# terra-render/Terra

Measured on AMD Instinct MI355X. Metric: Msamples/s, higher is better.
Workload: dtype f32; 1 GPU; cornell_1080p_512spp; scene=cornell32, width=1920, height=1080, spp=512, bounces=8, integrator=simple, triangles=32, tree=auto, traversal=reference tree + leaf-box cull, tile=64, sample_split=8, parallelism=single

## Files before the change

### terra_amd/csrc/integrators_device.h

```cpp
#pragma once
#include "shading_device.h"

TD float randf ( Pcg32& b, Counters& c, int count ) { if ( count == 2 ) ++c.rand_calls; return trng_b_float ( b ); }

TD float triangle_area ( V3 a, V3 b, V3 cc ) { return length ( cross ( b - a, cc - a ) ) / 2; }

struct LightSample { uint32_t light_object; uint32_t tri_in_object; uint32_t tri; float pick_pdf; V3 pos, norm; };

template <int COUNT, int MODE = 0>
TD LightSample draw_light_sample ( const DevScene& sc, Pcg32& rb, Counters& c, const Tracer* T = nullptr ) {
    LightSample ls;
    float e = ( float ) ( ( double ) randf ( rb, c, COUNT ) - 1e-4 );
    double xl = ( double ) e * ( double ) sc.n_lights;
    uint32_t li = xl < 0 ? 0u : ( uint32_t ) xl;
    ls.pick_pdf = 1.f / ( float ) sc.lights_triangles_count;
    DevLight l = ( MODE == 1 && T ) ? T->l_lights[li] : sc.lights[li];
    float e_t = randf ( rb, c, COUNT );
    uint32_t k = ( uint32_t ) ( e_t * ( float ) l.tri_count );
    if ( k >= l.tri_count ) k = l.tri_count - 1;
    ls.light_object = l.object; ls.tri_in_object = k; ls.tri = l.first_tri + k;
    float e1 = randf ( rb, c, COUNT ), e2 = randf ( rb, c, COUNT );
    const float4* tris = ( MODE == 1 && T ) ? reinterpret_cast<const float4*> ( T->l_tris ) : reinterpret_cast<const float4*> ( sc.tris );
    const float4* props = ( MODE == 1 && T ) ? T->l_props : reinterpret_cast<const float4*> ( sc.props );
    V3 ta, tb, tc; tri_vertices ( tris, ls.tri, ta, tb, tc );
// ... 279 lines not shown
    } else if ( INTEGRATOR == 2 ) {
        return integrate_mis<COUNT, MODE, KINDS, false> ( T, sf, p, wo, throughput, bounce, rb, c );
    } else if ( INTEGRATOR == 3 ) {
        return bounce != 0 ? v3 ( 0, 0, 0 ) : v3 ( 1, 1, 1 );
    } else if ( INTEGRATOR == 4 ) {
        if ( bounce != 0 ) return v3 ( 0, 0, 0 );
        float d = length ( ray.o - p ) / 500.f;
        return v3 ( d, d, d );
    } else if ( INTEGRATOR == 5 ) {
        return integrate_debug_normals ( sf, bounce );
    } else {
        return integrate_mis<COUNT, MODE, KINDS, true> ( T, sf, p, wo, throughput, bounce, rb, c );
    }
}

template <int COUNT>
TD PathDraws path_draw ( const float2* sincos24, Pcg32& rb, Counters& c ) {
    PathDraws d;
    d.e0 = randf ( rb, c, COUNT ); d.e1 = randf ( rb, c, COUNT ); d.e2 = randf ( rb, c, COUNT );
    d.az = azimuth_fetch ( sincos24, d.e1 );
    d.e3 = randf ( rb, c, COUNT );
    return d;
}
template <int KINDS>
TD bool path_continue ( Surface& sf, V3 wo, V3& throughput, uint32_t& bounce, uint32_t max_bounces, const PathDraws& d, V3& wi ) {
    wi = bsdf_sample<KINDS> ( sf, d.e0, d.e1, d.e2, wo, d.az );
    float pdf = sel_max ( bsdf_pdf<KINDS> ( sf, wi, wo ), ( float ) 1e-4 );
    V3 f = bsdf_eval<KINDS> ( sf, wi, wo ) * rcp_exact ( pdf );
    throughput = had ( throughput, f );
    throughput = throughput * dot ( sf.normal, wi );
    float pr = sel_max ( throughput.x, sel_max ( throughput.y, throughput.z ) );
    if ( d.e3 > pr ) return false;
        throughput = throughput * roulette_scale ( pr );
    ++bounce;
    return bounce <= max_bounces;
}
// ... 78 lines not shown
```

### terra_amd/csrc/render_kernels.hip

```cpp
#include <hip/hip_runtime.h>
#include "trace_device.h"
#include "kernels.h"
#include "launch_plan.h"
#include "empty_proof.h"

#ifdef TERRA_TU
#define TERRA_TU_HAS(k) ( TERRA_TU == ( k ) )
#define TERRA_TU_MODE(k) ( TERRA_TU == ( k ) || TERRA_TU == ( k ) + 4 || TERRA_TU == ( k ) + 8 || TERRA_TU == ( k ) + 12 )
#else
#define TERRA_TU_HAS(k) ( !TERRA_RAY_SOURCE )
#define TERRA_TU_MODE(k) 1
#endif
#if TERRA_RAY_SOURCE == 3
typedef DevPointRenderParams RenderKernelParams;
#elif TERRA_RAY_SOURCE == 2
typedef DevLensRenderParams RenderKernelParams;
#elif TERRA_RAY_SOURCE == 1
typedef DevRayRenderParams RenderKernelParams;
#else
typedef DevRenderParams RenderKernelParams;
#endif

struct DevResult { float acc[3]; int samples; };

// ... 612 lines not shown
    while ( true ) {
        const bool any_alive = __any ( alive );
        if ( !alive && ( TERRA_REGEN_MIN <= 1 || !any_alive || __popcll ( __ballot ( !alive ) ) >= TERRA_REGEN_MIN ) ) {
            if ( jb.s == p.chunk_spp && ( TERRA_JOB_FETCH_MIN <= 1 || !any_alive || __popcll ( __ballot ( jb.s == p.chunk_spp ) ) >= TERRA_JOB_FETCH_MIN ) ) TERRA_JOB_NEXT();
            if ( jb.exhausted ) break;
            if ( jb.s != p.chunk_spp ) {
                PS_WAVE ( c, kPsCamIter ); PS_LANE ( c, kPsCamLanes );
                float r1 = trng_a_float ( rs.a ), r2 = trng_a_float ( rs.a );
                TERRA_PRIMARY_RAY ( ro, rd, r1, r2 );
                if constexpr ( ( KINDS & TERRA_KIND_SAMPLER ) != 0 ) sp = sampler_pair_draw ( p.sampler_mode, p.sampler_strata, ( uint64_t ) jb.base + jb.s, rs.a );
                TERRA_LENS_RAY ( ro, rd, r1, r2 );
                lo_reset(); throughput = v3 ( 1, 1, 1 ); bounce = 0; alive = true; ++jb.s;
            }
        }
        if ( alive ) {
            ray = make_ray ( ro, rd );
            Surface sf;
            PS_WAVE ( c, kPsRayIter ); PS_LANE ( c, kPsRayLanes );
            constexpr bool pre_draw = !TERRA_IS_LIGHT ( INTEGRATOR );
            PathDraws pd;
            RaycastResult h = scene_raycast<COUNT, MODE, KINDS> ( T, ray, sf, c, pre_draw ? &pd : nullptr, pre_draw ? &rs.b : nullptr );
            bool end = !h.hit;
            if ( h.hit ) {
                PS_WAVE ( c, kPsShadeIter ); PS_LANE ( c, kPsShadeLanes );
                V3 wo = neg ( ray.d ), wi;
                constexpr bool SPLIT_DIRECT = INTEGRATOR == 1 && ( KINDS & ( TERRA_KIND_TEX | TERRA_KIND_SAMPLER ) ) == 0;
                if constexpr ( SPLIT_DIRECT ) {
                    Ray shadow_ray;
                    const DirectPending pend = direct_prepare<COUNT, KINDS, MODE> ( T, sf, h.point, wo, throughput, bounce, rs.b, c, shadow_ray );
                    pd = path_draw<COUNT> ( T.sc.sincos24, rs.b, c );
                    end = !path_continue<KINDS> ( sf, wo, throughput, bounce, p.bounces, pd, wi );
                    if ( !end ) { ro = surface_origin ( sf, h.point ); rd = wi; }
                    const uint32_t tri = scene_raycast_triangle<COUNT, MODE> ( T, shadow_ray, c, pend.expected );
                    lo_add ( tri == pend.expected ? pend.vis : pend.hid );
                } else if constexpr ( INTEGRATOR == 2 && ( KINDS & ( TERRA_KIND_TEX | TERRA_KIND_SAMPLER ) ) == 0 ) {
                    Ray ray_a; V3 b_d;
                    const MisPending pend = mis_prepare<COUNT, KINDS, MODE> ( T, sf, h.point, wo, throughput, bounce, rs.b, c, ray_a, b_d );
                    const V3 next_o = surface_origin ( sf, h.point );
                    end = !path_continue<COUNT, KINDS> ( T.sc, sf, wo, throughput, bounce, p.bounces, rs.b, c, wi, sp );
                    if ( !end ) { ro = next_o; rd = wi; }
                    const uint32_t tri_a = scene_raycast_triangle<COUNT, MODE> ( T, ray_a, c, pend.expected );
                    const V3 lo_a = tri_a == pend.expected ? pend.a_vis : pend.a_hid;
                    Surface lsf;
                    const RaycastResult hb = scene_raycast<COUNT, MODE, KINDS> ( T, make_ray ( next_o, b_d ), lsf, c );
                    lo_add ( mis_finish_b<MODE> ( T, pend, lo_a, hb.hit, hb.object, hb.tri, hb.point, lsf, b_d ) );
                } else {
                lo_add ( integrate<INTEGRATOR, COUNT, MODE, KINDS> ( T, ray, sf, h.point, wo, throughput, bounce, rs.b, c ) );
                if ( !pre_draw ) pd = path_draw<COUNT> ( T.sc.sincos24, rs.b, c );
                if constexpr ( ( KINDS & TERRA_KIND_SAMPLER ) != 0 ) path_apply_sampler ( pd, sp, bounce );
                end = !path_continue<KINDS> ( sf, wo, throughput, bounce, p.bounces, pd, wi );
                if ( !end ) { ro = surface_origin ( sf, h.point ); rd = wi; }
                }
            } else if ( ( KINDS & TERRA_KIND_ENV ) && T.sc.env_mode && !env_reaches_by_samples<INTEGRATOR, KINDS> ( T.sc, bounce ) ) {
                throughput = had ( throughput, environment_eval ( T.sc, ray.d ) );
                lo_add ( throughput );
            }
            if ( end ) { lo_deposit(); alive = false; }
        }
    }
    }

    if ( COUNT ) wave_flush_counters ( c, p.counters );
    if ( COUNT == 2 && p.leaf_cull ) {
// ... 309 lines not shown
```

### terra_amd/csrc/rng.h

```cpp
#pragma once
#include <stdint.h>

#if defined(__HIPCC__)
#define TRNG_FN __host__ __device__ inline
#else
#define TRNG_FN static inline
#endif

struct Pcg32 { uint64_t state, inc; };

TRNG_FN uint64_t trng_splitmix64 ( uint64_t z ) {
    z += 0x9E3779B97F4A7C15ull;
    z = ( z ^ ( z >> 30 ) ) * 0xBF58476D1CE4E5B9ull;
    z = ( z ^ ( z >> 27 ) ) * 0x94D049BB133111EBull;
    return z ^ ( z >> 31 );
}

TRNG_FN uint32_t trng_next ( Pcg32& g ) {
    uint64_t old = g.state;
    g.state = old * 6364136223846793005ull + g.inc;
    uint32_t xs = ( uint32_t ) ( ( ( old >> 18 ) ^ old ) >> 27 );
    uint32_t rot = ( uint32_t ) ( old >> 59 );
    return ( xs >> rot ) | ( xs << ( ( 0u - rot ) & 31u ) );
}
// ... 10 lines not shown

TRNG_FN PixelStreams trng_pixel_streams ( uint64_t frame_seed, uint64_t pix, uint64_t samples_so_far ) {
    PixelStreams s;
    uint64_t k = trng_splitmix64 ( trng_splitmix64 ( frame_seed + pix ) ^ ( samples_so_far * 0x9E3779B97F4A7C15ull ) );
    s.seedA = ( uint32_t ) ( k >> 32 );
    s.a.state = 0; s.a.inc = 1;
    trng_next ( s.a );
    s.a.state += s.seedA;
    trng_next ( s.a );
    trng_seed ( s.b, trng_splitmix64 ( k ^ 1ull ), trng_splitmix64 ( k ^ 2ull ) );
    return s;
}

TRNG_FN float trng_a_float ( Pcg32& a ) { return ( float ) trng_next ( a ) * 0x1p-32f; }
TRNG_FN float trng_b_float ( Pcg32& b ) { return ( float ) ( trng_next ( b ) >> 8 ) * 0x1p-24f; }
```

### terra_amd/csrc/shading_device.h

```cpp
#pragma once
#include "traverse_fast.h"

TD float texture_coord ( float u ) { return u > -1.f ? fminf ( u, 4294967040.f ) : 0.f; }
TD V3 texture_read ( const DevTexture& t, uint32_t x, uint32_t y ) {
    const uint32_t W = t.width, H = t.height;
    if ( t.address_mode == 2 ) { x = x < W - 1 ? x : W - 1; y = y < H - 1 ? y : H - 1; }
    else if ( t.address_mode == 0 ) { x %= W; y %= H; }
    else if ( ( x / W ) % 2 == 0 ) { x %= W; y %= H; }
    else { x = W - ( x % W ); y = H - ( y % H ); x = x < W - 1 ? x : W - 1; y = y < H - 1 ? y : H - 1; }
    const size_t e = ( ( size_t ) y * W + x ) * t.components;
    if ( t.depth == 1 ) {
        const uint8_t* p = reinterpret_cast<const uint8_t*> ( t.data ) + e;
        return v3 ( p[0] / 255.f, p[1] / 255.f, p[2] / 255.f );
    }
    const float* p = reinterpret_cast<const float*> ( t.data ) + e;
    return v3 ( p[0], p[1], p[2] );
}
TD V3 texture_sample ( const DevTexture& t, float u, float v ) {
    u = texture_coord ( u ); v = texture_coord ( v );
    uint32_t ix = ( uint32_t ) u, iy = ( uint32_t ) v;
    if ( t.filter == 0 ) return texture_read ( t, ix, iy );
    if ( t.filter != 1 ) return v3 ( 0, 0, 0 );
    uint32_t x2 = ix + 1 < t.width - 1 ? ix + 1 : t.width - 1, y2 = iy + 1 < t.height - 1 ? iy + 1 : t.height - 1;
    V3 n1 = texture_read ( t, ix, iy ), n2 = texture_read ( t, x2, iy ), n3 = texture_read ( t, ix, y2 ), n4 = texture_read ( t, x2, y2 );
// ... 73 lines not shown
        float tx = ( pc2.x * v + pb2.x * u ) + pa2.x * w;
        float ty = ( pc2.y * v + pb2.y * u ) + pa2.y * w;
        #pragma unroll
        for ( int i = 0; i < 4; ++i ) if ( m.tex[i] >= 0 ) sf.attr[i] = texture_sample ( T.sc.textures[m.tex[i]], tx, ty );
        if ( m.tex[TERRA_DEV_MAX_ATTR] >= 0 ) sf.emissive = texture_sample ( T.sc.textures[m.tex[TERRA_DEV_MAX_ATTR]], tx, ty );
    }
    sf.bsdf = m.bsdf;
    sf.ior = m.ior;
    nattr_out = m.attributes_count;
}

struct RaycastResult { bool hit; uint32_t object, tri_in_object, tri; V3 point; };

struct Azimuth { float sn, cs; bool have; };
struct PathDraws { float e0, e1, e2, e3; Azimuth az; };
template <int COUNT> TD PathDraws path_draw ( const float2* sincos24, Pcg32& rb, Counters& c );

template <int COUNT, int MODE, int KINDS>
TD RaycastResult scene_raycast ( const Tracer& T, const Ray& in, Surface& sf, Counters& c, PathDraws* pre = nullptr, Pcg32* rb = nullptr ) {
    Ray r = in;
    r.o = r.o + r.d * 0.001f;
    RayState st = ray_state_init ( r );
    if ( COUNT ) ++c.rays;
    Closest best;
    if ( MODE >= 2 ) { ClosestRanked b2 = bvh_traverse_fast<COUNT, MODE == 3> ( T, r, st, c ); best.depth = b2.depth; best.tri = b2.tri; }
    else best = bvh_traverse<COUNT, MODE> ( T, r, st, c );
    RaycastResult res; res.hit = best.tri != 0xffffffffu; res.tri = best.tri; res.object = 0; res.tri_in_object = 0;
    res.point = res.hit ? r.o + r.d * best.depth : v3 ( FLT_MAX, FLT_MAX, FLT_MAX );
    if ( res.hit ) {
        uint32_t nattr;
        if ( pre ) *pre = path_draw<COUNT> ( T.sc.sincos24, *rb, c );
        surface_init<MODE, KINDS> ( T, best.tri, res.point, sf, res.object, res.tri_in_object, nattr );
        if ( MODE >= 2 ) res.tri = T.sc.mats[res.object].first_tri + res.tri_in_object;
        if ( COUNT ) ++c.hits;
        if ( COUNT == 2 ) c.attr_fetches += nattr + 1;
    }
    return res;
}

template <int COUNT, int MODE>
TD uint32_t scene_raycast_triangle ( const Tracer& T, const Ray& in, Counters& c, uint32_t expected ) {
    Ray r = in;
    r.o = r.o + r.d * 0.001f;
    RayState st = ray_state_init ( r );
    if ( COUNT ) ++c.rays;
    if constexpr ( MODE == 2 && COUNT == 0 ) {
        const V3 o_perm = permuted ( r.o, st );
        ClosestRanked best;
        if ( !fast_expect ( T, st, o_perm, expected, best ) ) return 0xffffffffu;
        int* top = T.stack; uint32_t hand = TERRA_FAST_ROOT_IN_HAND, held = 0u;
        traverse_fast_resume<COUNT> ( T, r, st, o_perm, best, top, hand, held, 0, c, false, true );
        return best.tri == TERRA_TRI_EXPECTED ? expected : 0xffffffffu;
    }
    if constexpr ( MODE == 1 && COUNT == 0 ) {
        const V3 o_perm = permuted ( r.o, st );
        float depth;
        if ( !watertight_permuted ( tri_perm_lds ( T.l_tris + 12 * expected, st ), o_perm, st, depth ) ) return 0xffffffffu;
        Closest best; best.depth = __uint_as_float ( __float_as_uint ( depth + 0.f ) + 1u ); best.tri = 0xffffffffu;
        if ( T.pairs ) { best.depth = depth; best.tri = terra_pair_key ( __float_as_uint ( T.l_tris[12 * expected + 11] ), expected ); }
        if ( T.fused && __all ( ray_is_tame ( r ) ) ) traverse_loops<COUNT, MODE, true, true, true> ( T, r, st, o_perm, best, c, expected );
        else if ( __all ( ray_is_regular ( r ) ) ) traverse_loops<COUNT, MODE, true, false, true> ( T, r, st, o_perm, best, c, expected );
        else traverse_loops<COUNT, MODE, false, false, true> ( T, r, st, o_perm, best, c, expected );
        if ( T.pairs ) return best.tri != 0u ? expected : 0xffffffffu;
        return best.tri;
    }
    uint32_t tri;
    if ( MODE >= 2 ) { const ClosestRanked b2 = bvh_traverse_fast<COUNT, MODE == 3> ( T, r, st, c ); tri = b2.tri; }
    else tri = bvh_traverse<COUNT, MODE> ( T, r, st, c ).tri;
    if ( tri == 0xffffffffu ) return tri;
    uint32_t object;
// ... 9 lines not shown
    return tri;
}

TD V3 surface_origin ( const Surface& sf, V3 p ) { return p + sf.normal * 0.0001f; }
TD Ray surface_ray ( const Surface& sf, V3 p, V3 d ) { return make_ray ( surface_origin ( sf, p ), d ); }


TD Azimuth azimuth_none() { Azimuth a; a.sn = 0.f; a.cs = 1.f; a.have = false; return a; }
TD Azimuth azimuth_fetch ( const float2* tab, float e ) {
    Azimuth a = azimuth_none();
    const float x = e * 16777216.f;
    if ( tab && e >= 0.f && x < 16777216.f ) {
        const uint32_t k = ( uint32_t ) x;
        if ( ( float ) k == x ) { const float2 v = tab[k]; a.cs = v.x; a.sn = v.y; a.have = true; }
    }
    return a;
}
TD void azimuth_sincos ( const Azimuth& az, float e, float& sn, float& cs ) {
    if ( az.have ) { sn = az.sn; cs = az.cs; }
    else tdm_sincosf_pair ( 2 * TERRA_PI_F * e, sn, cs );
}

TD V3 diffuse_sample ( const Surface& sf, float e1, float e2, const Azimuth& az ) {
    float r = sqrt_exact ( e1 );
    float sn, cs;
    azimuth_sincos ( az, e2, sn, cs );
    float x = r * cs;
    float z = r * sn;
    V3 wi = v3 ( x, sqrt_exact ( sel_max ( 0.f, 1 - e1 ) ), z );
    return normalize ( basis_apply ( make_basis ( sf.normal ), wi ) );
// ... 145 lines not shown
```

### terra_amd/csrc/trace_geometry.h

```cpp
#pragma once
#include "trace_math.h"

TD void camera_film ( const DevRenderParams& p, uint32_t px, uint32_t py, float r1, float r2, float& sx, float& sy ) {
    float dx = -p.jitter + 2 * r1 * p.jitter;
    float dy = -p.jitter + 2 * r2 * p.jitter;
    float ndc_x, ndc_y; div2_exact_rk ( ( float ) px + 0.5f + dx, ( float ) py + 0.5f + dy, ( float ) p.fb_w, p.inv_fb_w, ( float ) p.fb_h, p.inv_fb_h, ndc_x, ndc_y );
    sx = 2 * ndc_x - 1;
    sy = 1 - 2 * ndc_y;
}
TD V3 camera_rotate ( const DevRenderParams& p, V3 d ) {
    return v3 ( p.cam_rot[0] * d.x + p.cam_rot[1] * d.y + p.cam_rot[2] * d.z,
                p.cam_rot[3] * d.x + p.cam_rot[4] * d.y + p.cam_rot[5] * d.z,
                p.cam_rot[6] * d.x + p.cam_rot[7] * d.y + p.cam_rot[8] * d.z );
}
TD V3 camera_sample ( const DevRenderParams& p, uint32_t px, uint32_t py, float r1, float r2 ) {
    float sx, sy; camera_film ( p, px, py, r1, r2, sx, sy );
    float fx = sx * p.aspect * p.tan_half_fov;
    float fy = sy * p.tan_half_fov;
    V3 d = normalize ( v3 ( fx, fy, 1.f ) );
    return camera_rotate ( p, d );
}

TD void concentric_disk ( float l1, float l2, float& u, float& v ) {
    const float kPi2 = tdm_float ( 0x3FC90FDBu ), kPi4 = tdm_float ( 0x3F490FDBu );
// ... 129 lines not shown
}

TD RayState ray_state_init ( const Ray& r ) {
    float ax = fabsf ( r.d.x ), ay = fabsf ( r.d.y ), az = fabsf ( r.d.z );
    int iz = ax > ay ? ( ax > az ? 0 : 2 ) : ( ay > az ? 1 : 2 );
    int ix = iz + 1 == 3 ? 0 : iz + 1;
    int iy = ix + 1 == 3 ? 0 : ix + 1;
    if ( pick ( r.d, iz ) < 0.f ) { int t = ix; ix = iy; iy = t; }
    RayState s;
    s.scalez = pick ( r.inv, iz );
    s.shearx = pick ( r.d, ix ) * s.scalez;
    s.sheary = pick ( r.d, iy ) * s.scalez;
    s.ix = ix; s.iy = iy; s.iz = iz;
    return s;
}

TD void tri_vertices ( float4 t0, float4 t1, float4 t2, V3& a, V3& b, V3& c ) { a = v3 ( t0.x, t0.y, t0.z ); b = v3 ( t1.x, t1.y, t1.z ); c = v3 ( t2.x, t2.y, t2.z ); }
TD void tri_vertices ( const float4* tris, uint32_t i, V3& a, V3& b, V3& c ) { tri_vertices ( tris[3 * i], tris[3 * i + 1], tris[3 * i + 2], a, b, c ); }

struct TriPerm { float a[3], b[3], c[3]; };
TD TriPerm tri_perm_lds ( const float* t, const RayState& s ) {
    TriPerm p;
    p.a[0] = t[s.ix]; p.a[1] = t[s.iy]; p.a[2] = t[s.iz];
    p.b[0] = t[4 + s.ix]; p.b[1] = t[4 + s.iy]; p.b[2] = t[4 + s.iz];
    p.c[0] = t[8 + s.ix]; p.c[1] = t[8 + s.iy]; p.c[2] = t[8 + s.iz];
    return p;
}
TD TriPerm tri_perm ( float4 t0, float4 t1, float4 t2, const RayState& s ) {
    const V3 va = v3 ( t0.x, t0.y, t0.z ), vb = v3 ( t1.x, t1.y, t1.z ), vc = v3 ( t2.x, t2.y, t2.z );
    TriPerm p;
// ... 138 lines not shown
```

### terra_amd/csrc/trace_math.h

```cpp
#pragma once
#include <hip/hip_runtime.h>
#include <float.h>
#include "dev_types.h"
#include "dev_math.h"
#include "rng.h"
#include "sampling_device.h"
#include "exact_div.h"
#include "exact_sqrt.h"

#define TD __device__ __forceinline__

struct V3 { float x, y, z; };

TD V3 v3 ( float x, float y, float z ) { V3 r; r.x = x; r.y = y; r.z = z; return r; }
TD V3 v3p ( const float* p ) { return v3 ( p[0], p[1], p[2] ); }
TD V3 operator+ ( V3 a, V3 b ) { return v3 ( a.x + b.x, a.y + b.y, a.z + b.z ); }
TD V3 operator- ( V3 a, V3 b ) { return v3 ( a.x - b.x, a.y - b.y, a.z - b.z ); }
TD V3 operator* ( V3 a, float s ) { return v3 ( a.x * s, a.y * s, a.z * s ); }
TD V3 had ( V3 a, V3 b ) { return v3 ( a.x * b.x, a.y * b.y, a.z * b.z ); }
TD V3 neg ( V3 a ) { return v3 ( -a.x, -a.y, -a.z ); }
TD float dot ( V3 a, V3 b ) { return a.x * b.x + a.y * b.y + a.z * b.z; }
TD V3 cross ( V3 a, V3 b ) { return v3 ( a.y * b.z - a.z * b.y, a.z * b.x - a.x * b.z, a.x * b.y - a.y * b.x ); }
TD float length2 ( V3 a ) { return a.x * a.x + a.y * a.y + a.z * a.z; }
TD float length ( V3 a ) { return sqrtf ( length2 ( a ) ); }
// ... 25 lines not shown
    } else {
        float k = sqrtf ( n.y * n.y + n.z * n.z );
        t = v3 ( 0.f * k, -n.z * k, n.y * k );
    }
    return basis_of ( t, n );
}
TD Basis make_basis ( V3 n ) {
    const bool c = fabsf ( n.x ) > fabsf ( n.y );
    const float a = c ? n.x : n.y;
    const float k = sqrt_exact ( a * a + n.z * n.z );
    return basis_of ( v3 ( ( c ? n.z : 0.f ) * k, ( c ? 0.f : -n.z ) * k, ( c ? -n.x : n.y ) * k ), n );
}

struct Ray { V3 o, d, inv; };
TD Ray make_ray ( V3 o, V3 d ) { Ray r; r.o = o; r.d = d; rcp3_exact ( d.x, d.y, d.z, r.inv.x, r.inv.y, r.inv.z ); return r; }

struct RayState { float shearx, sheary, scalez; int ix, iy, iz; };
TD V3 permuted ( V3 a, const RayState& s ) { return v3 ( pick ( a, s.ix ), pick ( a, s.iy ), pick ( a, s.iz ) ); }
```

### terra_amd/csrc/traverse_ref.h

```cpp
#pragma once
#include "trace_geometry.h"
#include <stddef.h>

#ifndef TERRA_PHASE_STATS
#define TERRA_PHASE_STATS 0
#endif
struct Counters {
    uint32_t rays, nodes, tri_tests, hits, rand_calls, attr_fetches;
    uint32_t tri_culled;
#if TERRA_PHASE_STATS
    uint32_t ps[16];
#endif
};
TD Counters counters_zero() {
    Counters c; c.rays = c.nodes = c.tri_tests = c.hits = c.rand_calls = c.attr_fetches = c.tri_culled = 0;
#if TERRA_PHASE_STATS
    for ( int i = 0; i < 16; ++i ) c.ps[i] = 0;
#endif
    return c;
}
#if TERRA_PHASE_STATS
#define PS_WAVE(c, k) do { if ( ( int ) ( threadIdx.x & 63 ) == __ffsll ( ( long long ) __ballot ( 1 ) ) - 1 ) ++( c ).ps[k]; } while ( 0 )
#define PS_LANE(c, k) do { ++( c ).ps[k]; } while ( 0 )
#else
// ... 164 lines not shown
    uint32_t sx = r.inv.x < 0.f ? kNeg : 0u, sy = r.inv.y < 0.f ? kNeg : 0u, sz = r.inv.z < 0.f ? kNeg : 0u;
    asm ( "" : "+v" ( sx ), "+v" ( sy ), "+v" ( sz ) );
    uint32_t bx = table + kX + sx, by = table + kY + sy, bz = table + kZ + sz;
    asm ( "" : "+v" ( bx ), "+v" ( by ), "+v" ( bz ) );
    const char* pm = reinterpret_cast<const char*> ( T.l_props ) + terra_leaf_box_mask_offset ( 0 );
    uint32_t leaf_set = 0u, entry = 0u;
    if constexpr ( PAIRS ) nb.lo = nb.hi = TERRA_NO_BOX;
    #pragma clang loop vectorize(disable) interleave(disable) unroll(disable)
    for ( uint32_t g = T.n_boxes / TERRA_LEAF_BOX_GROUP; g != 0; --g ) leaf_box_group<TERRA_LEAF_BOX_GROUP, kStride, PAIRS> ( bx, by, bz, pm, r, sel, leaf_set, c, entry, nb );
    if ( T.n_boxes & 4u ) leaf_box_group<4, kStride, PAIRS> ( bx, by, bz, pm, r, sel, leaf_set, c, entry, nb );
    #pragma clang loop vectorize(disable) interleave(disable) unroll(disable)
    for ( uint32_t k = T.n_boxes % 4u; k != 0; --k ) leaf_box_group<1, kStride, PAIRS> ( bx, by, bz, pm, r, sel, leaf_set, c, entry, nb );
    return leaf_set;
}

template <int COUNT, int MODE, bool FAST, bool FUSED, bool ANYHIT>
TD void traverse_pairs ( const Tracer& T, const Ray& r, const RayState& st, V3 o_perm, Closest& best, Counters& c ) {
    const SlabSel sel = slab_sel ( r );
    uint32_t leaf_set = 0u;
    PS_WAVE ( c, kPsDrainIter );
    bool flat = false;
    if constexpr ( FUSED ) flat = T.n_boxes != 0u;
    NearestBoxes nb; nb.lo = nb.hi = TERRA_NO_BOX;
    bool nearest = false;
    if ( flat ) { leaf_set = leaf_boxes_flat<true> ( T, r, sel, c, nb ); nearest = T.nearest; }
    else {
        int* sp = T.stack; int* lp = nullptr;
        *sp = 0; sp += TERRA_COL;
        while ( sp != T.stack ) node_step<COUNT, MODE, FAST, FUSED, true> ( T, r, sel, sp, lp, leaf_set, c );
    }
    const uint32_t perm = 2u * ( uint32_t ) st.iz + ( uint32_t ) ( st.ix != ( st.iz == 2 ? 0 : st.iz + 1 ) );
    const float4* copy = T.l_ranked + ( TERRA_PAIR_ENTRY_BYTES / 16 ) * ( T.lds_tris >> 1 ) * perm;
    float depth_best = best.depth; uint32_t key_best = ANYHIT ? best.tri : 0u;
    bool beaten = false;
    const float cut = __uint_as_float ( ( uint32_t ) ( nearest ? nb.hi : TERRA_NO_BOX ) & ~31u );
    if ( ANYHIT && nearest && depth_best < __uint_as_float ( ( uint32_t ) nb.lo & ~31u ) ) leaf_set = 0u;
    uint32_t next = nearest ? ( uint32_t ) nb.lo & 31u : ( uint32_t ) __builtin_ctz ( leaf_set | 0x80000000u );
    while ( leaf_set != 0u ) {
        PS_WAVE ( c, kPsLeafIter ); PS_LANE ( c, kPsLeafLanes );
        const float4* e = copy + ( TERRA_PAIR_ENTRY_BYTES / 16 ) * next;
        leaf_set &= ~ ( 1u << next );
        const uint2 keys = *reinterpret_cast<const uint2*> ( e + 3 );
        auto load = [&] ( bool again ) {
            uint32_t a = ( uint32_t ) ( uintptr_t ) e;
            if ( again ) asm volatile ( "" : "+v" ( a ) );
            typedef float Piece __attribute__ (( ext_vector_type ( 4 ) ));
// ... 3 lines not shown
        };
        watertight_pair ( load, o_perm, st, [&] ( float depth, bool second ) {
            const uint32_t key = second ? keys.y : keys.x;
            if ( ( depth < depth_best ) | ( ( depth == depth_best ) & ( key < key_best ) ) ) {
                if ( ANYHIT ) { beaten = true; leaf_set = 0u; }
                else { depth_best = depth; key_best = key; }
            }
        } );
        if ( depth_best < cut ) leaf_set = 0u;
        next = ( uint32_t ) __builtin_ctz ( leaf_set | 0x80000000u );
    }
    best.depth = depth_best;
    best.tri = ANYHIT ? ( beaten ? 0u : key_best ) : ( key_best ? ( key_best & 31u ) : 0xffffffffu );
}

template <int COUNT, int MODE, bool FAST, bool FUSED = false, bool ANYHIT = false>
TD void traverse_ranked ( const Tracer& T, const Ray& r, const RayState& st, V3 o_perm, Closest& best, Counters& c, uint32_t expected ) {
    if constexpr ( COUNT == 0 ) if ( T.pairs ) { traverse_pairs<COUNT, MODE, FAST, FUSED, ANYHIT> ( T, r, st, o_perm, best, c ); return; }
    const SlabSel sel = slab_sel ( r );
    uint32_t leaf_set = 0u;
    PS_WAVE ( c, kPsDrainIter );
    bool flat = false;
    if constexpr ( COUNT == 0 && FUSED ) flat = T.n_boxes != 0u;
    NearestBoxes no_nb;
    if ( flat ) leaf_set = leaf_boxes_flat<false> ( T, r, sel, c, no_nb );
    else {
        int* sp = T.stack; int* lp = nullptr;
        *sp = 0; sp += TERRA_COL;
        while ( sp != T.stack ) node_step<COUNT, MODE, FAST, FUSED, true> ( T, r, sel, sp, lp, leaf_set, c );
    }
    const uint32_t perm = 2u * ( uint32_t ) st.iz + ( uint32_t ) ( st.ix != ( st.iz == 2 ? 0 : st.iz + 1 ) );
    const float4* copy = T.l_ranked + 3u * T.lds_tris * perm;
    while ( leaf_set != 0u ) {
        PS_WAVE ( c, kPsLeafIter ); PS_LANE ( c, kPsLeafLanes );
        const float4* e = copy + 3u * ( uint32_t ) __builtin_ctz ( leaf_set );
        leaf_set &= leaf_set - 1u;
        const float4 q0 = e[0], q1 = e[1], q2 = e[2];
        const TriPerm tp = { { q0.x, q0.y, q0.z }, { q0.w, q1.x, q1.y }, { q1.z, q1.w, q2.x } };
        if ( COUNT ) ++c.tri_tests;
        float depth;
        if ( watertight_permuted ( tp, o_perm, st, depth ) && depth < best.depth ) {
            const uint32_t ti = __float_as_uint ( q2.y );
            best.depth = depth; best.tri = ti;
            if ( ANYHIT && ti != expected ) leaf_set = 0u;
        }
    }
}

template <int COUNT, int MODE, bool FAST, bool FUSED = false, bool ANYHIT = false>
TD void traverse_loops ( const Tracer& T, const Ray& r, const RayState& st, V3 o_perm, Closest& best, Counters& c, uint32_t expected = 0xffffffffu ) {
    if constexpr ( MODE == 1 ) if ( T.ranked ) { traverse_ranked<COUNT, MODE, FAST, FUSED, ANYHIT> ( T, r, st, o_perm, best, c, expected ); return; }
    const SlabSel sel = slab_sel ( r );
    int* sp = T.stack; int* lp = T.leaves;
    int* const lp_full = T.leaves + ( T.leaf_cap - 2 ) * TERRA_COL;
    uint32_t no_set = 0u;
    *sp = 0; sp += TERRA_COL;
    for ( ;; ) {
        PS_WAVE ( c, kPsDrainIter );
        while ( sp != T.stack && lp <= lp_full ) node_step<COUNT, MODE, FAST, FUSED> ( T, r, sel, sp, lp, no_set, c );
        if constexpr ( ANYHIT ) {
            bool stop = false;
            for ( const int* e = T.leaves; e != lp && !stop; e += TERRA_COL ) leaf_step<COUNT, MODE, true> ( T, e, st, o_perm, best, c, expected, &stop );
            if ( stop ) sp = T.stack;
        } else
        for ( const int* e = T.leaves; e != lp; e += TERRA_COL ) leaf_step<COUNT, MODE> ( T, e, st, o_perm, best, c );
        lp = T.leaves;
        if ( sp == T.stack ) break;
    }
}

template <int COUNT, int MODE>
TD Closest bvh_traverse ( const Tracer& T, const Ray& r, const RayState& st, Counters& c ) {
    Closest best; best.depth = FLT_MAX; best.tri = 0xffffffffu;
    V3 o_perm = permuted ( r.o, st );
    if ( MODE == 1 && T.fused && __all ( ray_is_tame ( r ) ) ) traverse_loops<COUNT, MODE, true, true> ( T, r, st, o_perm, best, c );
    else if ( __all ( ray_is_regular ( r ) ) ) traverse_loops<COUNT, MODE, true> ( T, r, st, o_perm, best, c );
    else traverse_loops<COUNT, MODE, false> ( T, r, st, o_perm, best, c );
    return best;
}

template <int COUNT, int MODE, bool FAST>
TD void traverse_resume ( const Tracer& T, const Ray& r, const SlabSel& sel, const RayState& st, V3 o_perm, Closest& best, int*& sp, bool& traversing, int exit_active, Counters& c ) {
    int* const lp_full = T.leaves + ( T.leaf_cap - 2 ) * TERRA_COL;
    int* lp = T.leaves;
    uint32_t no_set = 0u;
// ... 14 lines not shown
```

### terra_amd/csrc/unit_kernels.hip

```cpp
#include <hip/hip_runtime.h>
#include "trace_device.h"
#include "sampling_device.h"
#include "kernels.h"

#define UNIT_GRID(n) dim3 ( ( ( n ) + 255 ) / 256 ), dim3 ( 256 )

__global__ void k_pcg ( const uint32_t* seeds, int nseeds, int n, float* out ) {
    int i = blockIdx.x * blockDim.x + threadIdx.x;
    if ( i >= nseeds ) return;
    Pcg32 a; a.state = 0; a.inc = 1;
    trng_next ( a ); a.state += seeds[i]; trng_next ( a );
    for ( int j = 0; j < n; ++j ) out[ ( size_t ) i * n + j] = trng_a_float ( a );
}
hipError_t terra_unit_pcg ( const uint32_t* seeds, int nseeds, int n, float* out ) {
    hipLaunchKernelGGL ( k_pcg, UNIT_GRID ( nseeds ), 0, 0, seeds, nseeds, n, out );
    return hipGetLastError();
}

__global__ void k_stream_keys ( uint64_t seed, const uint64_t* pix, const uint64_t* k, int n, uint64_t* out3 ) {
    int i = blockIdx.x * blockDim.x + threadIdx.x;
    if ( i >= n ) return;
    PixelStreams s = trng_pixel_streams ( seed, pix[i], k[i] );
    out3[3 * i] = s.seedA; out3[3 * i + 1] = s.b.state; out3[3 * i + 2] = s.b.inc;
}
// ... 24 lines not shown
    TriHit h; h.u = h.v = h.w = h.depth = 0.f; h.point = v3 ( 0, 0, 0 );
    bool ok = watertight ( r, s, v3p ( tris + 9 * i ), v3p ( tris + 9 * i + 3 ), v3p ( tris + 9 * i + 6 ), h );
    hit[i] = ok ? 1 : 0;
    float* q = out8 + 8 * i;
    if ( ok ) { q[0] = h.u; q[1] = h.v; q[2] = h.w; q[3] = h.depth; q[4] = h.point.x; q[5] = h.point.y; q[6] = h.point.z; q[7] = 0.f; }
    else { for ( int j = 0; j < 8; ++j ) q[j] = 0.f; }
}
hipError_t terra_unit_watertight ( int n, const float* o, const float* d, const float* tris, int* hit, float* out8 ) {
    hipLaunchKernelGGL ( k_watertight, UNIT_GRID ( n ), 0, 0, n, o, d, tris, hit, out8 );
    return hipGetLastError();
}

__global__ void k_watertight_pair ( int n, const float* o, const float* d, const float* quads, int* hit, float* depth ) {
    int i = blockIdx.x * blockDim.x + threadIdx.x;
    if ( i >= n ) return;
    Ray r = make_ray ( v3p ( o + 3 * i ), v3p ( d + 3 * i ) );
    RayState s = ray_state_init ( r );
    auto load = [&] ( bool again ) {
        const float* q = quads + 12 * i;
        if ( again ) asm volatile ( "" : "+v" ( q ) );
        const V3 p0 = v3p ( q ), p1 = v3p ( q + 3 ), p2 = v3p ( q + 6 ), p3 = v3p ( q + 9 );
        return PairPerm { { pick ( p0, s.ix ), pick ( p0, s.iy ), pick ( p0, s.iz ) }, { pick ( p1, s.ix ), pick ( p1, s.iy ), pick ( p1, s.iz ) },
                          { pick ( p2, s.ix ), pick ( p2, s.iy ), pick ( p2, s.iz ) }, { pick ( p3, s.ix ), pick ( p3, s.iy ), pick ( p3, s.iz ) } };
    };
    int h0 = 0, h1 = 0; float d0 = 0.f, d1 = 0.f;
    watertight_pair ( load, permuted ( r.o, s ), s, [&] ( float dep, bool second ) { if ( second ) { h1 = 1; d1 = dep; } else { h0 = 1; d0 = dep; } } );
    hit[2 * i] = h0; hit[2 * i + 1] = h1; depth[2 * i] = d0; depth[2 * i + 1] = d1;
}
hipError_t terra_unit_watertight_pair ( int n, const float* o, const float* d, const float* quads, int* hit, float* depth ) {
    hipLaunchKernelGGL ( k_watertight_pair, UNIT_GRID ( n ), 0, 0, n, o, d, quads, hit, depth );
    return hipGetLastError();
}

__global__ void k_mt ( int n, const float* o, const float* d, const float* tris, int* hit, float* out4 ) {
    int i = blockIdx.x * blockDim.x + threadIdx.x;
    if ( i >= n ) return;
    float t = 0.f; V3 p = v3 ( 0, 0, 0 );
    bool ok = moller_trumbore ( v3p ( o + 3 * i ), v3p ( d + 3 * i ), v3p ( tris + 9 * i ), v3p ( tris + 9 * i + 3 ), v3p ( tris + 9 * i + 6 ), t, p );
    hit[i] = ok ? 1 : 0;
    out4[4 * i] = ok ? t : 0.f; out4[4 * i + 1] = ok ? p.x : 0.f; out4[4 * i + 2] = ok ? p.y : 0.f; out4[4 * i + 3] = ok ? p.z : 0.f;
}
// ... 417 lines not shown
```

Before: 36180 Msamples/s.

## Compute ray permutation via select masks and guarded fast reciprocals

Adds a ray-setup path for camera rays in the fused mode. It builds the watertight permutation state with boolean selects and a packed permutation code, and produces the permuted origin directly. It also computes direction reciprocals with a short reciprocal when a range check passes, so the traversal can skip the wave-wide tame/regular checks. The azimuth table lookup now uses the integer random bits instead of converting float back to an index. The change adds code paths and template variants, and the results depend on the short reciprocal matching the exact one closely enough.

New measurement: 37030 Msamples/s (median of 6 runs). 1.02x the previous value.

```diff
diff --git a/terra_amd/csrc/integrators_device.h b/terra_amd/csrc/integrators_device.h
--- a/terra_amd/csrc/integrators_device.h
+++ b/terra_amd/csrc/integrators_device.h
@@ -2,6 +2,7 @@
 #include "shading_device.h"
 
 TD float randf ( Pcg32& b, Counters& c, int count ) { if ( count == 2 ) ++c.rand_calls; return trng_b_float ( b ); }
+TD uint32_t randf_bits ( Pcg32& b, Counters& c, int count ) { if ( count == 2 ) ++c.rand_calls; return trng_b_bits ( b ); }
 
 TD float triangle_area ( V3 a, V3 b, V3 cc ) { return length ( cross ( b - a, cc - a ) ) / 2; }
 
@@ -317,12 +318,21 @@
     }
 }
 
-template <int COUNT>
+template <int COUNT, bool INDEX>
 TD PathDraws path_draw ( const float2* sincos24, Pcg32& rb, Counters& c ) {
     PathDraws d;
-    d.e0 = randf ( rb, c, COUNT ); d.e1 = randf ( rb, c, COUNT ); d.e2 = randf ( rb, c, COUNT );
-    d.az = azimuth_fetch ( sincos24, d.e1 );
-    d.e3 = randf ( rb, c, COUNT );
+    if constexpr ( INDEX ) {
+        d.e0 = randf ( rb, c, COUNT );
+        const uint32_t k1 = randf_bits ( rb, c, COUNT );
+        d.e1 = trng_b_from_bits ( k1 );
+        d.e2 = randf ( rb, c, COUNT );
+        d.az = azimuth_fetch_index ( sincos24, k1 );
+        d.e3 = randf ( rb, c, COUNT );
+    } else {
+        d.e0 = randf ( rb, c, COUNT ); d.e1 = randf ( rb, c, COUNT ); d.e2 = randf ( rb, c, COUNT );
+        d.az = azimuth_fetch ( sincos24, d.e1 );
+        d.e3 = randf ( rb, c, COUNT );
+    }
     return d;
 }
 template <int KINDS>
diff --git a/terra_amd/csrc/render_kernels.hip b/terra_amd/csrc/render_kernels.hip
--- a/terra_amd/csrc/render_kernels.hip
+++ b/terra_amd/csrc/render_kernels.hip
@@ -650,12 +650,14 @@
             }
         }
         if ( alive ) {
+            bool guarded = false;
+            if constexpr ( ray_start_masks_for ( COUNT, MODE, KINDS ) ) ray = make_ray_guarded ( ro, rd, guarded ); else
             ray = make_ray ( ro, rd );
             Surface sf;
             PS_WAVE ( c, kPsRayIter ); PS_LANE ( c, kPsRayLanes );
             constexpr bool pre_draw = !TERRA_IS_LIGHT ( INTEGRATOR );
             PathDraws pd;
-            RaycastResult h = scene_raycast<COUNT, MODE, KINDS> ( T, ray, sf, c, pre_draw ? &pd : nullptr, pre_draw ? &rs.b : nullptr );
+            RaycastResult h = scene_raycast<COUNT, MODE, KINDS> ( T, ray, sf, c, pre_draw ? &pd : nullptr, pre_draw ? &rs.b : nullptr, guarded );
             bool end = !h.hit;
             if ( h.hit ) {
                 PS_WAVE ( c, kPsShadeIter ); PS_LANE ( c, kPsShadeLanes );
@@ -664,10 +666,10 @@
                 if constexpr ( SPLIT_DIRECT ) {
                     Ray shadow_ray;
                     const DirectPending pend = direct_prepare<COUNT, KINDS, MODE> ( T, sf, h.point, wo, throughput, bounce, rs.b, c, shadow_ray );
-                    pd = path_draw<COUNT> ( T.sc.sincos24, rs.b, c );
+                    pd = path_draw<COUNT, ray_start_masks_for ( COUNT, MODE, KINDS )> ( T.sc.sincos24, rs.b, c );
                     end = !path_continue<KINDS> ( sf, wo, throughput, bounce, p.bounces, pd, wi );
                     if ( !end ) { ro = surface_origin ( sf, h.point ); rd = wi; }
-                    const uint32_t tri = scene_raycast_triangle<COUNT, MODE> ( T, shadow_ray, c, pend.expected );
+                    const uint32_t tri = scene_raycast_triangle<COUNT, MODE, ray_start_masks_for ( COUNT, MODE, KINDS )> ( T, shadow_ray, c, pend.expected );
                     lo_add ( tri == pend.expected ? pend.vis : pend.hid );
                 } else if constexpr ( INTEGRATOR == 2 && ( KINDS & ( TERRA_KIND_TEX | TERRA_KIND_SAMPLER ) ) == 0 ) {
                     Ray ray_a; V3 b_d;
@@ -675,14 +677,14 @@
                     const V3 next_o = surface_origin ( sf, h.point );
                     end = !path_continue<COUNT, KINDS> ( T.sc, sf, wo, throughput, bounce, p.bounces, rs.b, c, wi, sp );
                     if ( !end ) { ro = next_o; rd = wi; }
-                    const uint32_t tri_a = scene_raycast_triangle<COUNT, MODE> ( T, ray_a, c, pend.expected );
+                    const uint32_t tri_a = scene_raycast_triangle<COUNT, MODE, ray_start_masks_for ( COUNT, MODE, KINDS )> ( T, ray_a, c, pend.expected );
                     const V3 lo_a = tri_a == pend.expected ? pend.a_vis : pend.a_hid;
                     Surface lsf;
                     const RaycastResult hb = scene_raycast<COUNT, MODE, KINDS> ( T, make_ray ( next_o, b_d ), lsf, c );
                     lo_add ( mis_finish_b<MODE> ( T, pend, lo_a, hb.hit, hb.object, hb.tri, hb.point, lsf, b_d ) );
                 } else {
                 lo_add ( integrate<INTEGRATOR, COUNT, MODE, KINDS> ( T, ray, sf, h.point, wo, throughput, bounce, rs.b, c ) );
-                if ( !pre_draw ) pd = path_draw<COUNT> ( T.sc.sincos24, rs.b, c );
+                if ( !pre_draw ) pd = path_draw<COUNT, ray_start_masks_for ( COUNT, MODE, KINDS )> ( T.sc.sincos24, rs.b, c );
                 if constexpr ( ( KINDS & TERRA_KIND_SAMPLER ) != 0 ) path_apply_sampler ( pd, sp, bounce );
                 end = !path_continue<KINDS> ( sf, wo, throughput, bounce, p.bounces, pd, wi );
                 if ( !end ) { ro = surface_origin ( sf, h.point ); rd = wi; }
diff --git a/terra_amd/csrc/rng.h b/terra_amd/csrc/rng.h
--- a/terra_amd/csrc/rng.h
+++ b/terra_amd/csrc/rng.h
@@ -48,3 +48,5 @@
 
 TRNG_FN float trng_a_float ( Pcg32& a ) { return ( float ) trng_next ( a ) * 0x1p-32f; }
 TRNG_FN float trng_b_float ( Pcg32& b ) { return ( float ) ( trng_next ( b ) >> 8 ) * 0x1p-24f; }
+TRNG_FN uint32_t trng_b_bits ( Pcg32& b ) { return trng_next ( b ) >> 8; }
+TRNG_FN float trng_b_from_bits ( uint32_t k ) { return ( float ) k * 0x1p-24f; }
diff --git a/terra_amd/csrc/shading_device.h b/terra_amd/csrc/shading_device.h
--- a/terra_amd/csrc/shading_device.h
+++ b/terra_amd/csrc/shading_device.h
@@ -111,22 +111,26 @@
 
 struct Azimuth { float sn, cs; bool have; };
 struct PathDraws { float e0, e1, e2, e3; Azimuth az; };
-template <int COUNT> TD PathDraws path_draw ( const float2* sincos24, Pcg32& rb, Counters& c );
+template <int COUNT, bool INDEX = false> TD PathDraws path_draw ( const float2* sincos24, Pcg32& rb, Counters& c );
 
 template <int COUNT, int MODE, int KINDS>
-TD RaycastResult scene_raycast ( const Tracer& T, const Ray& in, Surface& sf, Counters& c, PathDraws* pre = nullptr, Pcg32* rb = nullptr ) {
+TD RaycastResult scene_raycast ( const Tracer& T, const Ray& in, Surface& sf, Counters& c, PathDraws* pre = nullptr, Pcg32* rb = nullptr, bool guarded = false ) {
     Ray r = in;
     r.o = r.o + r.d * 0.001f;
-    RayState st = ray_state_init ( r );
+    constexpr bool MASKS = ray_start_masks_for ( COUNT, MODE, KINDS );
     if ( COUNT ) ++c.rays;
     Closest best;
+    if constexpr ( MASKS ) { V3 o_perm; const RayStateMasks st = ray_start_masks ( r, o_perm ); best = bvh_traverse_from<COUNT, MODE> ( T, r, st, o_perm, c, __all ( guarded ) != 0 ); }
+    else {
+    RayState st = ray_state_init ( r );
     if ( MODE >= 2 ) { ClosestRanked b2 = bvh_traverse_fast<COUNT, MODE == 3> ( T, r, st, c ); best.depth = b2.depth; best.tri = b2.tri; }
     else best = bvh_traverse<COUNT, MODE> ( T, r, st, c );
+    }
     RaycastResult res; res.hit = best.tri != 0xffffffffu; res.tri = best.tri; res.object = 0; res.tri_in_object = 0;
     res.point = res.hit ? r.o + r.d * best.depth : v3 ( FLT_MAX, FLT_MAX, FLT_MAX );
     if ( res.hit ) {
         uint32_t nattr;
-        if ( pre ) *pre = path_draw<COUNT> ( T.sc.sincos24, *rb, c );
+        if ( pre ) *pre = path_draw<COUNT, MASKS> ( T.sc.sincos24, *rb, c );
         surface_init<MODE, KINDS> ( T, best.tri, res.point, sf, res.object, res.tri_in_object, nattr );
         if ( MODE >= 2 ) res.tri = T.sc.mats[res.object].first_tri + res.tri_in_object;
         if ( COUNT ) ++c.hits;
@@ -135,11 +139,12 @@
     return res;
 }
 
-template <int COUNT, int MODE>
+template <int COUNT, int MODE, bool MASKS = false>
 TD uint32_t scene_raycast_triangle ( const Tracer& T, const Ray& in, Counters& c, uint32_t expected ) {
     Ray r = in;
     r.o = r.o + r.d * 0.001f;
-    RayState st = ray_state_init ( r );
+    V3 o_masks = v3 ( 0, 0, 0 );
+    const auto st = [&] { if constexpr ( MASKS ) return ray_start_masks ( r, o_masks ); else return ray_state_init ( r ); } ();
     if ( COUNT ) ++c.rays;
     if constexpr ( MODE == 2 && COUNT == 0 ) {
         const V3 o_perm = permuted ( r.o, st );
@@ -150,7 +155,7 @@
         return best.tri == TERRA_TRI_EXPECTED ? expected : 0xffffffffu;
     }
     if constexpr ( MODE == 1 && COUNT == 0 ) {
-        const V3 o_perm = permuted ( r.o, st );
+        const V3 o_perm = MASKS ? o_masks : permuted ( r.o, st );
         float depth;
         if ( !watertight_permuted ( tri_perm_lds ( T.l_tris + 12 * expected, st ), o_perm, st, depth ) ) return 0xffffffffu;
         Closest best; best.depth = __uint_as_float ( __float_as_uint ( depth + 0.f ) + 1u ); best.tri = 0xffffffffu;
@@ -190,6 +195,11 @@
         const uint32_t k = ( uint32_t ) x;
         if ( ( float ) k == x ) { const float2 v = tab[k]; a.cs = v.x; a.sn = v.y; a.have = true; }
     }
+    return a;
+}
+TD Azimuth azimuth_fetch_index ( const float2* tab, uint32_t k ) {
+    Azimuth a = azimuth_none();
+    if ( tab ) { const float2 v = tab[k]; a.cs = v.x; a.sn = v.y; a.have = true; }
     return a;
 }
 TD void azimuth_sincos ( const Azimuth& az, float e, float& sn, float& cs ) {
diff --git a/terra_amd/csrc/trace_geometry.h b/terra_amd/csrc/trace_geometry.h
--- a/terra_amd/csrc/trace_geometry.h
+++ b/terra_amd/csrc/trace_geometry.h
@@ -167,6 +167,34 @@
     s.ix = ix; s.iy = iy; s.iz = iz;
     return s;
 }
+
+TD RayStateMasks ray_start_masks ( const Ray& r, V3& o_perm ) {
+    const float ax = fabsf ( r.d.x ), ay = fabsf ( r.d.y ), az = fabsf ( r.d.z );
+    const bool xy = ax > ay, xz = ax > az, yz = ay > az;
+    const bool z0 = xy & xz, z1 = !xy & yz;
+    const auto at_z = [&] ( V3 a ) { return z0 ? a.x : ( z1 ? a.y : a.z ); };
+    const bool flip = at_z ( r.d ) < 0.f;
+    const auto at_xy = [&] ( V3 a, float& px, float& py ) {
+        const float u = z0 ? a.y : ( z1 ? a.z : a.x ), v = z0 ? a.z : ( z1 ? a.x : a.y );
+        px = flip ? v : u; py = flip ? u : v;
+    };
+    RayStateMasks s;
+    s.perm = ( z0 ? 0u : ( z1 ? 2u : 4u ) ) + ( flip ? 1u : 0u );
+    asm volatile ( "" : "+v" ( s.perm ) );
+    s.ix = ( int ) ( ( 0x429u >> ( 2u * s.perm ) ) & 3u ); s.iy = ( int ) ( ( 0x186u >> ( 2u * s.perm ) ) & 3u ); s.iz = ( int ) ( s.perm >> 1 );
+    s.scalez = at_z ( r.inv );
+    float dix, diy; at_xy ( r.d, dix, diy );
+    s.shearx = dix * s.scalez;
+    s.sheary = diy * s.scalez;
+    at_xy ( r.o, o_perm.x, o_perm.y ); o_perm.z = at_z ( r.o );
+    return s;
+}
+#if TERRA_RAY_SOURCE
+#define TERRA_RAY_START_CAMERA 0
+#else
+#define TERRA_RAY_START_CAMERA 1
+#endif
+TD constexpr bool ray_start_masks_for ( int COUNT, int MODE, int KINDS ) { return TERRA_RAY_START_CAMERA && MODE == 1 && COUNT == 0 && KINDS == 1; }
 
 TD void tri_vertices ( float4 t0, float4 t1, float4 t2, V3& a, V3& b, V3& c ) { a = v3 ( t0.x, t0.y, t0.z ); b = v3 ( t1.x, t1.y, t1.z ); c = v3 ( t2.x, t2.y, t2.z ); }
 TD void tri_vertices ( const float4* tris, uint32_t i, V3& a, V3& b, V3& c ) { tri_vertices ( tris[3 * i], tris[3 * i + 1], tris[3 * i + 2], a, b, c ); }
diff --git a/terra_amd/csrc/trace_math.h b/terra_amd/csrc/trace_math.h
--- a/terra_amd/csrc/trace_math.h
+++ b/terra_amd/csrc/trace_math.h
@@ -63,6 +63,16 @@
 
 struct Ray { V3 o, d, inv; };
 TD Ray make_ray ( V3 o, V3 d ) { Ray r; r.o = o; r.d = d; rcp3_exact ( d.x, d.y, d.z, r.inv.x, r.inv.y, r.inv.z ); return r; }
+TD Ray make_ray_guarded ( V3 o, V3 d, bool& guarded ) {
+    Ray r; r.o = o; r.d = d;
+    guarded = ( xd_rcp_ok ( d.x ) & xd_rcp_ok ( d.y ) & xd_rcp_ok ( d.z ) ) != 0;
+    if ( guarded ) { r.inv.x = xd_rcp_short ( d.x ); r.inv.y = xd_rcp_short ( d.y ); r.inv.z = xd_rcp_short ( d.z ); }
+    else { r.inv.x = 1.f / d.x; r.inv.y = 1.f / d.y; r.inv.z = 1.f / d.z; }
+    return r;
+}
 
 struct RayState { float shearx, sheary, scalez; int ix, iy, iz; };
 TD V3 permuted ( V3 a, const RayState& s ) { return v3 ( pick ( a, s.ix ), pick ( a, s.iy ), pick ( a, s.iz ) ); }
+TD uint32_t ray_perm ( const RayState& s ) { return 2u * ( uint32_t ) s.iz + ( uint32_t ) ( s.ix != ( s.iz == 2 ? 0 : s.iz + 1 ) ); }
+struct RayStateMasks : RayState { uint32_t perm; };
+TD uint32_t ray_perm ( const RayStateMasks& s ) { return s.perm; }
diff --git a/terra_amd/csrc/traverse_ref.h b/terra_amd/csrc/traverse_ref.h
--- a/terra_amd/csrc/traverse_ref.h
+++ b/terra_amd/csrc/traverse_ref.h
@@ -202,8 +202,8 @@
     return leaf_set;
 }
 
-template <int COUNT, int MODE, bool FAST, bool FUSED, bool ANYHIT>
-TD void traverse_pairs ( const Tracer& T, const Ray& r, const RayState& st, V3 o_perm, Closest& best, Counters& c ) {
+template <int COUNT, int MODE, bool FAST, bool FUSED, bool ANYHIT, class RS = RayState>
+TD void traverse_pairs ( const Tracer& T, const Ray& r, const RS& st, V3 o_perm, Closest& best, Counters& c ) {
     const SlabSel sel = slab_sel ( r );
     uint32_t leaf_set = 0u;
     PS_WAVE ( c, kPsDrainIter );
@@ -217,7 +217,7 @@
         *sp = 0; sp += TERRA_COL;
         while ( sp != T.stack ) node_step<COUNT, MODE, FAST, FUSED, true> ( T, r, sel, sp, lp, leaf_set, c );
     }
-    const uint32_t perm = 2u * ( uint32_t ) st.iz + ( uint32_t ) ( st.ix != ( st.iz == 2 ? 0 : st.iz + 1 ) );
+    const uint32_t perm = ray_perm ( st );
     const float4* copy = T.l_ranked + ( TERRA_PAIR_ENTRY_BYTES / 16 ) * ( T.lds_tris >> 1 ) * perm;
     float depth_best = best.depth; uint32_t key_best = ANYHIT ? best.tri : 0u;
     bool beaten = false;
@@ -251,8 +251,8 @@
     best.tri = ANYHIT ? ( beaten ? 0u : key_best ) : ( key_best ? ( key_best & 31u ) : 0xffffffffu );
 }
 
-template <int COUNT, int MODE, bool FAST, bool FUSED = false, bool ANYHIT = false>
-TD void traverse_ranked ( const Tracer& T, const Ray& r, const RayState& st, V3 o_perm, Closest& best, Counters& c, uint32_t expected ) {
+template <int COUNT, int MODE, bool FAST, bool FUSED = false, bool ANYHIT = false, class RS = RayState>
+TD void traverse_ranked ( const Tracer& T, const Ray& r, const RS& st, V3 o_perm, Closest& best, Counters& c, uint32_t expected ) {
     if constexpr ( COUNT == 0 ) if ( T.pairs ) { traverse_pairs<COUNT, MODE, FAST, FUSED, ANYHIT> ( T, r, st, o_perm, best, c ); return; }
     const SlabSel sel = slab_sel ( r );
     uint32_t leaf_set = 0u;
@@ -266,7 +266,7 @@
         *sp = 0; sp += TERRA_COL;
         while ( sp != T.stack ) node_step<COUNT, MODE, FAST, FUSED, true> ( T, r, sel, sp, lp, leaf_set, c );
     }
-    const uint32_t perm = 2u * ( uint32_t ) st.iz + ( uint32_t ) ( st.ix != ( st.iz == 2 ? 0 : st.iz + 1 ) );
+    const uint32_t perm = ray_perm ( st );
     const float4* copy = T.l_ranked + 3u * T.lds_tris * perm;
     while ( leaf_set != 0u ) {
         PS_WAVE ( c, kPsLeafIter ); PS_LANE ( c, kPsLeafLanes );
@@ -284,8 +284,8 @@
     }
 }
 
-template <int COUNT, int MODE, bool FAST, bool FUSED = false, bool ANYHIT = false>
-TD void traverse_loops ( const Tracer& T, const Ray& r, const RayState& st, V3 o_perm, Closest& best, Counters& c, uint32_t expected = 0xffffffffu ) {
+template <int COUNT, int MODE, bool FAST, bool FUSED = false, bool ANYHIT = false, class RS = RayState>
+TD void traverse_loops ( const Tracer& T, const Ray& r, const RS& st, V3 o_perm, Closest& best, Counters& c, uint32_t expected = 0xffffffffu ) {
     if constexpr ( MODE == 1 ) if ( T.ranked ) { traverse_ranked<COUNT, MODE, FAST, FUSED, ANYHIT> ( T, r, st, o_perm, best, c, expected ); return; }
     const SlabSel sel = slab_sel ( r );
     int* sp = T.stack; int* lp = T.leaves;
@@ -306,6 +306,15 @@
     }
 }
 
+template <int COUNT, int MODE, class RS>
+TD Closest bvh_traverse_from ( const Tracer& T, const Ray& r, const RS& st, V3 o_perm, Counters& c, bool all_guarded ) {
+    Closest best; best.depth = FLT_MAX; best.tri = 0xffffffffu;
+    const bool guarded = all_guarded;
+    if ( MODE == 1 && T.fused && ( guarded || __all ( ray_is_tame ( r ) ) ) ) traverse_loops<COUNT, MODE, true, true> ( T, r, st, o_perm, best, c );
+    else if ( guarded || __all ( ray_is_regular ( r ) ) ) traverse_loops<COUNT, MODE, true> ( T, r, st, o_perm, best, c );
+    else traverse_loops<COUNT, MODE, false> ( T, r, st, o_perm, best, c );
+    return best;
+}
 template <int COUNT, int MODE>
 TD Closest bvh_traverse ( const Tracer& T, const Ray& r, const RayState& st, Counters& c ) {
     Closest best; best.depth = FLT_MAX; best.tri = 0xffffffffu;
diff --git a/terra_amd/csrc/unit_kernels.hip b/terra_amd/csrc/unit_kernels.hip
--- a/terra_amd/csrc/unit_kernels.hip
+++ b/terra_amd/csrc/unit_kernels.hip
@@ -62,8 +62,10 @@
 __global__ void k_watertight_pair ( int n, const float* o, const float* d, const float* quads, int* hit, float* depth ) {
     int i = blockIdx.x * blockDim.x + threadIdx.x;
     if ( i >= n ) return;
-    Ray r = make_ray ( v3p ( o + 3 * i ), v3p ( d + 3 * i ) );
-    RayState s = ray_state_init ( r );
+    bool guarded;
+    Ray r = make_ray_guarded ( v3p ( o + 3 * i ), v3p ( d + 3 * i ), guarded );
+    V3 o_perm;
+    const RayStateMasks s = ray_start_masks ( r, o_perm );
     auto load = [&] ( bool again ) {
         const float* q = quads + 12 * i;
         if ( again ) asm volatile ( "" : "+v" ( q ) );
@@ -72,7 +74,7 @@
                           { pick ( p2, s.ix ), pick ( p2, s.iy ), pick ( p2, s.iz ) }, { pick ( p3, s.ix ), pick ( p3, s.iy ), pick ( p3, s.iz ) } };
     };
     int h0 = 0, h1 = 0; float d0 = 0.f, d1 = 0.f;
-    watertight_pair ( load, permuted ( r.o, s ), s, [&] ( float dep, bool second ) { if ( second ) { h1 = 1; d1 = dep; } else { h0 = 1; d0 = dep; } } );
+    watertight_pair ( load, o_perm, s, [&] ( float dep, bool second ) { if ( second ) { h1 = 1; d1 = dep; } else { h0 = 1; d0 = dep; } } );
     hit[2 * i] = h0; hit[2 * i + 1] = h1; depth[2 * i] = d0; depth[2 * i + 1] = d1;
 }
 hipError_t terra_unit_watertight_pair ( int n, const float* o, const float* d, const float* quads, int* hit, float* depth ) {
```
